# sisl/MADRL

Hardware: AMD Instinct MI355X
Metric: env-steps/sec at fixed batch (PursuitEvade 16x16, 8v30) (higher is better)
Workload: dtype u8/int32 grid state, f32 observations, f64 reward arithmetic; 1 GPU; PursuitEvade 16x16, 8 pursuers / 30 evaders, obs_range 7, rectangle_map, surround, n_catch 2, flatten, local reward, 65536 envs per GPU, horizon 500; envs_per_gpu=65536, envs_total=65536, parallelism=env-sharded x1, streams_per_gpu=2, rccl_ranks=1

## Files before the change

madrl_amd/csrc/pursuit_wave.hpp:

```cpp
#pragma once

#include <type_traits>

#include "common.hpp"
#include "pursuit_rules.hpp"
#include "pursuit_zm16.hpp"

namespace madrl {
namespace pw {

#ifndef MADRL_PW_WAVES
#define MADRL_PW_WAVES 5
#endif
#define MADRL_PW_OCC __attribute__((amdgpu_waves_per_eu(S::OCC, S::OCC)))

constexpr uint32_t SENT = 0xFFFFFFFFu;
constexpr uint32_t CAUGHT = 0x10000u;

struct WaveDev {
    int32_t n_catch, surround, reward_global, sample_maps, n_maps, max_steps, auto_reset;
    int32_t fmap_stride;
    int32_t max_opponents;
    int32_t reverse;
    uint32_t k0, k1, gid_base;
    double catchr, term_pursuit, urgency, cw;
    int64_t n_envs;
    const uint32_t *fmaps;
    const float *vtab;
    const int32_t *pending;
    const uint32_t *cnt_tmpl;
    const uint32_t *slot_tab;
    const double *cw_env;
    const double *catchr_env;
    uint8_t *state;
    uint32_t *flags;
    uint32_t *zmask;
};

struct WaveIO {
    const uint8_t *mask;
    const int32_t *inj_pos;
    const int32_t *inj_map;
    const int32_t *actions;
    const int32_t *inj_eact;
    float *obs;
    float *rew;
    uint8_t *done;
    int32_t *removed;
    int32_t flex;
    int32_t control_evaders;
    const float *obs_prev;
};

__device__ __forceinline__ double sload_f64(const double *p, int64_t index) {
    return ((const __attribute__((address_space(4))) double *)(uint64_t)p)[index];
}

struct KArgs {
    WaveDev d;
    WaveIO io;
};
typedef const __attribute__((address_space(4))) KArgs *KArgsPtr;
__device__ __forceinline__ KArgsPtr cold_args() { return kernargs<KArgs>(); }
__device__ __forceinline__ int32_t pending_count(int64_t env, int k) {
    const int32_t *pend = cold_args()->d.pending;
    return ((const __attribute__((address_space(4))) int32_t *)(uint64_t)pend)[2 * env + k];
}

template <int XS_, int YS_, int P_, int E_, int R_, int FLATTEN_>
struct Shape {
    static constexpr int XS = XS_, YS = YS_, P = P_, E = E_, A = P_ + E_, R = R_, FLATTEN = FLATTEN_;
    static constexpr int OFF = (R - 1) / 2;
    static constexpr int PAD = OFF > 1 ? OFF : 1;
    static constexpr int GW = YS + 2 * PAD;
    static constexpr int GH = XS + 2 * PAD;
    static constexpr int GSZ = (GH * GW + 3) / 4 * 4;
    static constexpr int D = FLATTEN ? 3 * R * R + 1 : 4 * R * R;
    static constexpr int DV = D / 4;
    static constexpr int NQ = P * DV;
    static constexpr int NS = (NQ + 63) / 64;
    static constexpr int MWORDS = 1;
    static constexpr bool ZM16 = zm16::eligible(P, R, FLATTEN);
    static constexpr int ZMW = ZM16 ? 32 : 64;
    static constexpr int OCC = NS <= 5 ? MADRL_PW_WAVES : (MADRL_PW_WAVES < 4 ? MADRL_PW_WAVES : 4);
    static constexpr int X_FILL = 3 * GSZ;
    static constexpr int X_SKIP = 3 * GSZ + 1;
    static constexpr int X_ID = 3 * GSZ + 2;
    static constexpr int X_VTAB = (X_ID + P + 3) / 4 * 4;
    static constexpr int NVT = 72;
    static constexpr int X_NEED = X_VTAB + NVT;
    static constexpr int X_OBSV = X_NEED + (XS * YS + 3) / 4;
    static constexpr int LDS_DWORDS = X_OBSV + (P + 3) / 4 * 4;
    static constexpr int NGW = (E + 31) / 32 > 0 ? (E + 31) / 32 : 1;
    static constexpr int NTW = (A + 31) / 32;
    static constexpr int OFF_GONE = (16 + 2 * A + 3) / 4 * 4;
    static constexpr int OFF_TERM = OFF_GONE + 4 * NGW;
    static constexpr int REC_BYTES = (OFF_TERM + 4 * NTW + 15) / 16 * 16;
    static constexpr int REC_DW = REC_BYTES / 4;
    static_assert(REC_DW <= 64, "the whole record must fit one dword per lane");
    static_assert(A <= 64, "one wavefront per env: n_pursuers + n_evaders must fit 64 lanes");
    static_assert(R % 2 == 1, "odd obs_range only (even ranges run on the generic kernel)");
    static_assert(D % 4 == 0, "observation row must be a whole number of float4");
    static_assert(LDS_DWORDS * 4 <= 64 * 1024, "LDS budget");
    static_assert(NS <= 8, "stale-zero mask: one bit per slot in each byte of the lane's mask dword");
    static constexpr bool LIVE = false;
    static constexpr bool TO = false;
    static constexpr bool H16 = false;
    static constexpr bool LEAN_REGS = false;
    static constexpr bool TABLED = false;
    static constexpr int X_TAB = 0;
};

template <int XS_, int YS_, int P_, int E_, int R_, int FLATTEN_>
struct LShape : Shape<XS_, YS_, P_, E_, R_, FLATTEN_> {
    static constexpr bool LIVE = true;
};
constexpr int NOT_HERE = 0xFF;

template <int XS_, int YS_, int P_, int E_, int R_, int FLATTEN_>
struct TShape : Shape<XS_, YS_, P_, E_, R_, FLATTEN_> {
    static constexpr bool TO = true;
};
template <int XS_, int YS_, int P_, int E_, int R_, int FLATTEN_>
struct TLShape : LShape<XS_, YS_, P_, E_, R_, FLATTEN_> {
    static constexpr bool TO = true;
};
template <int XS_, int YS_, int P_, int E_, int R_, int FLATTEN_>
struct THShape : Shape<XS_, YS_, P_, E_, R_, FLATTEN_> {
    static constexpr bool TO = true;
    static constexpr bool H16 = true;
    static constexpr bool LEAN_REGS = true;
};
template <int XS_, int YS_, int P_, int E_, int R_, int FLATTEN_>
struct TLHShape : LShape<XS_, YS_, P_, E_, R_, FLATTEN_> {
    static constexpr bool TO = true;
    static constexpr bool H16 = true;
    static constexpr bool LEAN_REGS = true;
};

__device__ __forceinline__ double pairwise8(const double *r) {
    return ((r[0] + r[1]) + (r[2] + r[3])) + ((r[4] + r[5]) + (r[6] + r[7]));
}

template <int P>
__device__ __forceinline__ double np_sum_regs(const double (&a)[P]) {
    if constexpr (P < 8) {
        double res = 0.0;
#pragma unroll
        for (int i = 0; i < P; ++i) res += a[i];
        return res;
    } else {
        double r[8];
#pragma unroll
        for (int i = 0; i < 8; ++i) r[i] = a[i];
        constexpr int LIM = P - (P % 8);
#pragma unroll
        for (int i = 8; i < LIM; i += 8) {
#pragma unroll
            for (int k = 0; k < 8; ++k) r[k] += a[i + k];
        }
        double res = pairwise8(r);
#pragma unroll
        for (int i = LIM; i < P; ++i) res += a[i];
        return res;
    }
}

template <int P>
__device__ __forceinline__ double np_sum_first(const double (&a)[P], int n) {
    double res = 0.0;
    if (n < 8) {
#pragma unroll
        for (int i = 0; i < (P < 8 ? P : 7); ++i)
            if (i < n) res += a[i];
        return res;
    }
    if constexpr (P >= 8) {
        double r[8];
#pragma unroll
        for (int i = 0; i < 8; ++i) r[i] = a[i];
        const int lim = n - (n % 8);
#pragma unroll
        for (int i = 8; i + 8 <= P; i += 8) {
            if (i < lim) {
#pragma unroll
                for (int k = 0; k < 8; ++k) r[k] += a[i + k];
            }
        }
        res = pairwise8(r);
#pragma unroll
        for (int i = 8; i < P; ++i)
            if (i >= lim && i < n) res += a[i];
    }
    return res;
}

typedef float v4f_t __attribute__((ext_vector_type(4)));
template <int I, int N, class F>
__device__ __forceinline__ void static_for(F &&f) {
    if constexpr (I < N) {
        f(std::integral_constant<int, I>{});
        static_for<I + 1, N>(f);
    }
}
template <int OFF, bool H16 = false>
__device__ __forceinline__ void store_slot_masked(const void *base, uint32_t voff, uint32_t v0, uint32_t v1, uint32_t v2, uint32_t v3,
                                                  v4f_t val, uint64_t m0, uint64_t m1, uint64_t m2, uint64_t m3, uint64_t m_nt) {
    static_assert(!H16, "store_slot_masked is float32 geometry: an H16 shape runs its in-place pass through half_slot_in_place");
    uint64_t sv;
    asm volatile("s_mov_b64 %0, exec\n\t"
                 "s_mov_b64 exec, %1\n\tglobal_store_dword %6, %7, %12 offset:%13\n\t"
                 "s_mov_b64 exec, %2\n\tglobal_store_dword %6, %8, %12 offset:%13+4\n\t"
                 "s_mov_b64 exec, %3\n\tglobal_store_dword %6, %9, %12 offset:%13+8\n\t"
                 "s_mov_b64 exec, %4\n\tglobal_store_dword %6, %10, %12 offset:%13+12\n\t"
                 "s_mov_b64 exec, %5\n\tglobal_store_dwordx4 %6, %11, %12 offset:%13 nt\n\t"
                 "s_mov_b64 exec, %0\n\ts_nop 0"
                 : "=&s"(sv) : "s"(m0), "s"(m1), "s"(m2), "s"(m3), "s"(m_nt), "v"(voff), "v"(v0), "v"(v1), "v"(v2), "v"(v3), "v"(val),
                   "s"(base), "n"(OFF));
}
__device__ __forceinline__ uint32_t quad_or(uint32_t v) {
    v |= (uint32_t)__builtin_amdgcn_update_dpp(0, (int)v, 0xB1, 0xF, 0xF, true);
    v |= (uint32_t)__builtin_amdgcn_update_dpp(0, (int)v, 0x4E, 0xF, 0xF, true);
    return v;
}

__device__ __forceinline__ void prefetch3(uint32_t &r0, uint32_t &r1, uint32_t &r2, const void *b0, uint32_t o0, const void *b1, uint32_t o1,
                                          const void *b2, uint32_t o2) {
    asm volatile("s_nop 4\n\tglobal_load_dword %0, %3, %4\n\tglobal_load_dword %1, %5, %6\n\tglobal_load_dword %2, %7, %8"
                 : "=&v"(r0), "=&v"(r1), "=&v"(r2) : "v"(o0), "s"(b0), "v"(o1), "s"(b1), "v"(o2), "s"(b2));
}
template <int N>
__device__ __forceinline__ void prefetch_wait(uint32_t &r0, uint32_t &r1, uint32_t &r2) {
    static_assert(N >= 0 && N < 64, "vmcnt is a 6-bit field");
    asm volatile("s_waitcnt vmcnt(%3)" : "+v"(r0), "+v"(r1), "+v"(r2) : "n"(N) : "memory");
}

template <class RowPtr>
__device__ __forceinline__ void half_slot_in_place(RowPtr row, uint32_t slot, bool valid, uint32_t keep4, uint32_t v0, uint32_t v1, uint32_t v2,
                                                   uint32_t v3) {
    typedef __attribute__((address_space(1))) uint64_t gu64_t;
    if (!valid) return;
    auto hb = [](uint32_t v) -> uint64_t { return half_bits(__uint_as_float((uint32_t)max((int)v, 0))); };
    uint64_t w = hb(v0) | (hb(v1) << 16) | (hb(v2) << 32) | (hb(v3) << 48);
    gu64_t *const at = reinterpret_cast<gu64_t *>(row) + slot;
    if (keep4 != 0u) {
        const uint64_t old = __hip_atomic_load(at, __ATOMIC_RELAXED, __HIP_MEMORY_SCOPE_AGENT);
        const uint64_t k = ((keep4 & 0x00000001u) ? 0x000000000000FFFFull : 0ull) | ((keep4 & 0x00000100u) ? 0x00000000FFFF0000ull : 0ull) |
                           ((keep4 & 0x00010000u) ? 0x0000FFFF00000000ull : 0ull) | ((keep4 & 0x01000000u) ? 0xFFFF000000000000ull : 0ull);
        w = (w & ~k) | (old & k);
    }
    *at = w;
}

template <int LN>
__device__ __forceinline__ void put_lane(uint32_t &w, uint32_t v) {
    const uint32_t sv = (uint32_t)__builtin_amdgcn_readfirstlane((int)v);
    asm("v_writelane_b32 %0, %1, %2" : "+v"(w) : "s"(sv), "n"(LN));
}
template <int LN, int END>
__device__ __forceinline__ void put_zero_from(uint32_t &w) {
    if constexpr (LN < END) {
        put_lane<LN>(w, 0u);
        put_zero_from<LN + 1, END>(w);
    }
}

template <class S, int NT>
struct Fill {
    static constexpr int NEEDW = (S::XS * S::YS + 3) / 4;
    static constexpr int TABW = S::TABLED ? 2 * S::DV : 0;
    static constexpr int J_MAP = (S::GSZ + NT - 1) / NT;
    static constexpr int J_NEED = 2 * J_MAP;
    static constexpr int J_VT = J_NEED + (NEEDW + NT - 1) / NT;
    static constexpr int J_TAB = J_VT + (S::NVT + NT - 1) / NT;
    static constexpr int J_END = J_TAB + (TABW + NT - 1) / NT;
    static constexpr int first(int j) { return j < J_MAP ? 0 : j < J_NEED ? J_MAP : j < J_VT ? J_NEED : j < J_TAB ? J_VT : J_TAB; }
    static constexpr int words(int j) { return j < J_NEED ? S::GSZ : j < J_VT ? NEEDW : j < J_TAB ? S::NVT : TABW; }
};
template <class S, int NT, int J>
__device__ __forceinline__ uint32_t fill_load(uint32_t utid, const uint32_t *cnt, const uint32_t *map, const uint32_t *vtab, const uint32_t *tab) {
    using F = Fill<S, NT>;
    constexpr int t = J - F::first(J), n = F::words(J);
    const uint32_t k = utid + (uint32_t)(NT * t);
    const uint32_t kc = (NT * (t + 1) <= n) ? k : (k < (uint32_t)n ? k : (uint32_t)n - 1u);
    if constexpr (J < F::J_MAP) return cnt[kc];
    else if constexpr (J < F::J_NEED) return map[kc];
    else if constexpr (J < F::J_VT) return map[(uint32_t)S::GSZ + kc];
    else if constexpr (J < F::J_TAB) return vtab[kc];
    else return tab[kc];
}
template <class S, int NT, int J, bool FIRST>
__device__ __forceinline__ void fill_store(uint32_t *L, uint32_t utid, uint32_t v) {
    using F = Fill<S, NT>;
    constexpr int t = J - F::first(J), n = F::words(J);
    const uint32_t k = utid + (uint32_t)(NT * t);
    if ((NT * (t + 1) <= n) || k < (uint32_t)n) {
        if constexpr (J < F::J_MAP) {
            L[S::GSZ + k] = v;
            L[2 * S::GSZ + k] = v;
        } else if constexpr (J < F::J_NEED) L[k] = v;
        else if constexpr (J < F::J_VT) L[S::X_NEED + k] = v;
        else if constexpr (J < F::J_TAB) L[S::X_VTAB + k] = v;
        else L[S::X_TAB + k] = v;
    }
    if constexpr (FIRST && J == F::J_MAP) {
        if (utid == 0u) {
            L[S::X_FILL] = v;
            L[S::X_SKIP] = SENT;
        }
    }
}
template <int N>
__device__ __forceinline__ void staged_wait(uint32_t *a) {
    if constexpr (N >= 8) {
        asm volatile("" : "+v"(a[N - 1]), "+v"(a[N - 2]), "+v"(a[N - 3]), "+v"(a[N - 4]), "+v"(a[N - 5]), "+v"(a[N - 6]), "+v"(a[N - 7]), "+v"(a[N - 8]));
        staged_wait<N - 8>(a);
    } else if constexpr (N >= 4) {
        asm volatile("" : "+v"(a[N - 1]), "+v"(a[N - 2]), "+v"(a[N - 3]), "+v"(a[N - 4]));
        staged_wait<N - 4>(a);
    } else if constexpr (N >= 2) {
        asm volatile("" : "+v"(a[N - 1]), "+v"(a[N - 2]));
        staged_wait<N - 2>(a);
    } else if constexpr (N == 1) {
        asm volatile("" : "+v"(a[0]));
    }
}
template <class S, int NT, int J0, int J1, int CAP, bool FIRST>
__device__ __forceinline__ void fill_trips(uint32_t *L, uint32_t utid, const uint32_t *cnt, const uint32_t *map, const uint32_t *vtab, const uint32_t *tab) {
    if constexpr (J0 < J1) {
        constexpr int JB = J0 + CAP < J1 ? J0 + CAP : J1;
        uint32_t st[JB - J0];
        static_for<J0, JB>([&](auto jc) {
            if constexpr (decltype(jc)::value == JB - 1) __builtin_amdgcn_sched_barrier(0);
            st[decltype(jc)::value - J0] = fill_load<S, NT, decltype(jc)::value>(utid, cnt, map, vtab, tab);
        });
        staged_wait<JB - J0>(st);
        static_for<J0, JB>([&](auto jc) { fill_store<S, NT, decltype(jc)::value, FIRST>(L, utid, st[decltype(jc)::value - J0]); });
        fill_trips<S, NT, JB, J1, CAP, FIRST>(L, utid, cnt, map, vtab, tab);
    }
}
constexpr int FILL_FIRST = 56, FILL_BATCH = 16;

#ifndef MADRL_ABLATE
#define MADRL_ABLATE 0
#endif
#ifndef MADRL_PW_EXP
#define MADRL_PW_EXP 0
#endif

template <class S, int MODE, bool INJECT, bool CTRL = false>
__global__ __launch_bounds__(64) MADRL_PW_OCC void pursuit_wave_kernel(const WaveDev d, const WaveIO io) {
    static_assert(!CTRL || (S::E >= S::P && (MODE == 0 || INJECT)), "evader control: n_evaders >= n_pursuers, flexible instantiation");
    static_assert(!CTRL || !S::LIVE, "evader control has no per-env agent counts");
    static_assert(!S::TO || (MODE == 1 && INJECT && !CTRL), "the two-buffer step: the flexible step kernel only");
    static_assert(!S::H16 || S::TO, "binary16 buffers: the two-buffer step only");
    constexpr int P = S::P, E = S::E, A = S::A, GW = S::GW, PAD = S::PAD, GSZ = S::GSZ, NS = S::NS;
    __shared__ __attribute__((aligned(16))) uint32_t L[S::LDS_DWORDS];
    const int lane = threadIdx.x;
    const uint32_t ulane = threadIdx.x;
    const bool is_p = lane < P;
    const int eslot = lane - P;

#if MADRL_PW_EXP & 4
    if (d.n_envs > 0) return;
#endif
    using F = Fill<S, 64>;
    const int n_envs = (int)d.n_envs, stride = (int)gridDim.x;
    if (n_envs <= 0) return;
    auto phys = [&](int e) -> int64_t { return (int64_t)(d.reverse ? n_envs - 1 - e : e); };
    auto zm_env = [](int64_t env) -> int64_t { return (MADRL_ABLATE & (256 | 512)) ? (env & 255) : env; };
    const uint32_t zm_lane = S::ZM16 ? (ulane & 31u) : ulane;
    [[maybe_unused]] const uint32_t zm_keep = S::ZM16 ? zm16::keep_low(P, S::R, lane) : 0u;
    const uint32_t *const vtab_u = reinterpret_cast<const uint32_t *>(d.vtab);
    constexpr int ROOM = FILL_FIRST - 6 * NS - 3;
    constexpr int JF = F::J_END < (ROOM > 4 ? ROOM : 4) ? F::J_END : (ROOM > 4 ? ROOM : 4);
    const uint32_t rec_off = (ulane < (uint32_t)S::REC_DW ? ulane : (uint32_t)S::REC_DW - 1u) * 4u;
    const uint32_t act_off = (ulane < (uint32_t)P ? ulane : (uint32_t)P - 1u) * 4u;
    uint32_t st[JF], sraw[6 * NS];
    static_for<0, JF>([&](auto jc) { st[decltype(jc)::value] = fill_load<S, 64, decltype(jc)::value>(ulane, d.cnt_tmpl, d.fmaps, vtab_u, nullptr); });
#pragma unroll
    for (int k = 0; k < 6 * NS; ++k) sraw[k] = d.slot_tab[64u * k + ulane];
    uint32_t cur_rec, cur_zm;
    int cur_act = 4;
    __builtin_amdgcn_sched_barrier(0);
    {
        const int64_t env0 = phys((int)blockIdx.x < n_envs ? (int)blockIdx.x : n_envs - 1);
        cur_rec = *reinterpret_cast<const uint32_t *>(d.state + env0 * (int64_t)S::REC_BYTES + rec_off);
        if constexpr (MODE == 1) cur_act = *reinterpret_cast<const int *>(reinterpret_cast<const char *>(io.actions + env0 * P) + act_off);
        cur_zm = d.zmask[zm_env(env0) * S::ZMW + zm_lane];
    }
    asm volatile("" : "+v"(cur_rec), "+v"(cur_act), "+v"(cur_zm));
    staged_wait<6 * NS>(sraw);
    staged_wait<JF>(st);
    static_for<0, JF>([&](auto jc) { fill_store<S, 64, decltype(jc)::value, true>(L, ulane, st[decltype(jc)::value]); });
    fill_trips<S, 64, JF, F::J_END, FILL_BATCH, true>(L, ulane, d.cnt_tmpl, d.fmaps, vtab_u, nullptr);
    if (lane < P) L[S::X_ID + lane] = __float_as_uint((float)((double)lane / (double)P));
    if (ulane >= (uint32_t)S::REC_DW) cur_rec = 0u;
    if (!is_p) cur_act = 4;
    int s_cst[NS][4];
    int s_rel3[NS];
    int s_src[NS];
#pragma unroll
    for (int s = 0; s < NS; ++s) {
#pragma unroll
        for (int k = 0; k < 4; ++k) s_cst[s][k] = (int)sraw[6 * s + k] * 4;
        s_rel3[s] = (int)sraw[6 * s + 4];
        s_src[s] = (int)sraw[6 * s + 5] * 4;
    }
    int cached_map = 0;
    int cached_np = P;
    const uint8_t *need_tab = reinterpret_cast<const uint8_t *>(&L[S::X_NEED]);
    uint32_t *const layer = &L[is_p ? GSZ : 2 * GSZ];
    const int rec_src0 = (lane >= 4 ? 2 * (lane - 4) : 0) * 4, rec_src1 = rec_src0 + 4;

    auto isP = [&]() { return fresh(lane) < P; };
    auto isE = [&]() { return (unsigned)(fresh(lane) - P) < (unsigned)E; };
    auto isAgent = [&]() { return fresh(lane) < A; };
    auto fetch_rec = [&](int64_t env) -> uint32_t {
        return (fresh(lane) < S::REC_DW) ? uniform_ptr(reinterpret_cast<const uint32_t *>(d.state + env * (int64_t)S::REC_BYTES))[ulane] : 0u;
    };
    auto fetch_act = [&](int64_t env) -> int {
        if constexpr (MODE == 1) return isP() ? uniform_ptr(io.actions + env * P)[ulane] : 4;
        else return 4;
    };
    auto fetch_zm = [&](int64_t env) -> uint32_t {
        if constexpr (S::LEAN_REGS) return uniform_ptr(d.zmask + zm_env(env) * S::ZMW)[S::ZM16 ? ((uint32_t)fresh(lane) & 31u) : (uint32_t)fresh(lane)];
        else return uniform_ptr(d.zmask + zm_env(env) * S::ZMW)[zm_lane];
    };
    wave_sync();
#if MADRL_PW_EXP & 8
    if (d.n_envs > 0) { if (s_cst[0][0] + s_cst[NS - 1][3] + s_rel3[0] + s_src[NS - 1] + (int)cur_rec == 0x12345) io.rew[0] = 1.f; return; }
#endif

    constexpr bool PIPE = (MODE == 1) && !INJECT && !(MADRL_ABLATE & (1 | 8 | 16 | 64));
    constexpr int VM_PER_ENV = 5 * NS + 6 - ((MADRL_ABLATE & 512) ? 1 : 0);
    static_assert(!PIPE || VM_PER_ENV < 64, "vmcnt range");
    for (int e = blockIdx.x; e < n_envs; e += stride) {
        const int64_t env = phys(e);
        const bool has_next = e + stride < n_envs;
        const int64_t nenv = phys(has_next ? e + stride : e);
        uint32_t nxt_rec = 0, nxt_zm = 0xFFFFFFFFu;
        int nxt_act = 4;
        uint32_t pf_rec, pf_act, pf_zm;
        if constexpr (PIPE) {
            prefetch3(pf_rec, pf_act, pf_zm, d.state + nenv * (int64_t)S::REC_BYTES, rec_off, io.actions + nenv * P, act_off,
                      d.zmask + zm_env(nenv) * S::ZMW, zm_lane * 4u);
        } else {
#if MADRL_ABLATE & 64
            nxt_rec = cur_rec ^ (uint32_t)(fresh(lane) == 0);
            nxt_act = cur_act;
#else
            if (has_next) {
                nxt_rec = fetch_rec(nenv);
                nxt_act = fetch_act(nenv);
                nxt_zm = fetch_zm(nenv);
            }
#endif
        }
        bool skip = false;
        if constexpr (MODE == 0) skip = (io.mask != nullptr && io.mask[env] == 0);
        if (!skip) {
            uint32_t tick = __builtin_amdgcn_readlane(cur_rec, 0);
            int32_t tstep = (int32_t)__builtin_amdgcn_readlane(cur_rec, 1);
            int32_t map_id = (int32_t)__builtin_amdgcn_readlane(cur_rec, 2);
            const uint32_t xyw = (uint32_t)__shfl((int)cur_rec, 4 + (lane >> 1));
            const pr::Cell at = pr::unpack_xy(xyw, lane & 1);
            int x = at.x, y = at.y;
            uint64_t gone = (uint32_t)__builtin_amdgcn_readlane(cur_rec, S::OFF_GONE / 4);
            if constexpr (S::NGW > 1) gone |= (uint64_t)(uint32_t)__builtin_amdgcn_readlane(cur_rec, S::OFF_GONE / 4 + 1) << 32;
            uint64_t term = (uint32_t)__builtin_amdgcn_readlane(cur_rec, S::OFF_TERM / 4);
            if constexpr (S::NTW > 1) term |= (uint64_t)(uint32_t)__builtin_amdgcn_readlane(cur_rec, S::OFF_TERM / 4 + 1) << 32;
            const uint32_t gid = d.gid_base + (uint32_t)env;
            const uint32_t k0 = fresh_s(d.k0), k1 = fresh_s(d.k1);
            int np = P, ne = E;
            if constexpr (S::LIVE) {
                const bool here = x != NOT_HERE;
                np = __popcll(__builtin_amdgcn_ballot_w64(isP() && here));
                ne = __popcll(__builtin_amdgcn_ballot_w64(isE() && here));
                if (!here) {
                    x = 0;
                    y = 0;
                }
            }
            auto isLP = [&]() {
                if constexpr (S::LIVE) return fresh(lane) < np;
                else return isP();
            };
            bool do_reset = (MODE == 0);
            uint32_t done_bits = 0;
            float rew_out = 0.0f;
            int n_removed = 0;
            bool alive = isLP() || (isE() && !((gone >> eslot) & 1ull));
            int cell = (x + PAD) * GW + y + PAD;

            auto load_map = [&](int mid) {
                if (cached_map == mid) return;
                const KArgsPtr ka = cold_args();
                fill_trips<S, 64, F::J_MAP, F::J_VT, FILL_BATCH, false>(L, ulane, nullptr, ka->d.fmaps + (int64_t)mid * ka->d.fmap_stride, nullptr, nullptr);
                cached_map = mid;
                wave_sync();
            };
            load_map(map_id);

            if constexpr (MODE == 1) {
                const bool e_alive = alive && !isP();
                if (e_alive) atomicAdd(&layer[cell], 1u);
                wave_sync();
                int kpre = 0;
                if (isP()) {
                    const pr::Clip4 n = pr::clipped_neighbours<GW, S::XS, S::YS>(x, y);
                    const uint32_t *ec = &L[2 * GSZ];
                    kpre = (int)(ec[cell - n.dxm] + ec[cell + n.dxp] + ec[cell + n.dyp] + ec[cell - n.dym]);
                }
                wave_sync();
                if (e_alive) atomicSub(&layer[cell], 1u);
                const int kidx = __popcll((~gone) & ((1ull << (eslot & 63)) - 1ull));
                int act = cur_act;
                bool injected = false;
                if constexpr (CTRL) {
                    const int from_k = __builtin_amdgcn_ds_bpermute((kidx < P ? kidx : 0) * 4, cur_act);
                    injected = io.inj_eact != nullptr;
                    int pact;
                    if (injected) pact = isP() ? io.inj_eact[env * P + lane] : 4;
                    else pact = pr::pursuer_action(gid, tick, (uint32_t)lane, k0, k1);
                    act = isP() ? pact : (kidx < P ? from_k : 4);
                    injected = true;
                } else if constexpr (INJECT) {
                    injected = io.inj_eact != nullptr;
                    if (injected && e_alive) act = io.inj_eact[env * E + kidx];
                }
                if (!injected) {
#if MADRL_ABLATE & 4
                    u32x4 r; r.x = (gid * 2654435761u + tick * 40503u + (uint32_t)kidx * 2246822519u) ^ k0 ^ k1;
#else
                    const u32x4 r = philox4x32_10(gid, tick, (uint32_t)kidx, TAG_EVADER_ACT, k0, k1);
#endif
                    if (!isP()) act = (int)__umulhi(r.x, 5u);
                }
                const int dcell = pr::move_dcell<GW>(act);
                const bool tflag = (term >> lane) & 1ull;
                const bool in_building = L[cell] != 0u;
                const bool target_free = L[cell + dcell] == 0u;
                const bool newterm = alive && !tflag && in_building;
                if (alive && !tflag && !in_building && target_free) {
                    cell += dcell;
                    x += pr::move_dx(act), y += pr::move_dy(act);
                }
                term |= __ballot(newterm);
                if (alive) atomicAdd(&layer[cell], 1u);
                wave_sync();
                bool caught = false;
                if (e_alive) {
                    const uint32_t *pc = &L[GSZ];
                    if (d.surround) caught = pr::cells_with_pursuers(pc[cell - GW], pc[cell + GW], pc[cell + 1], pc[cell - 1], SENT) == (int)need_tab[x * S::YS + y];
                    else caught = (int)pc[cell] >= d.n_catch;
                    if (caught) atomicAdd(&layer[cell], CAUGHT);
                }
                const uint64_t caught_mask = __ballot(caught) >> P;
                gone |= caught_mask;
                wave_sync();
                double r = 0.0;
                if (isLP()) {
                    const uint32_t *ec = &L[2 * GSZ];
                    bool sur;
                    if (d.surround) sur = pr::caught_beside(ec[cell - GW], ec[cell + GW], ec[cell + 1], ec[cell - 1], SENT, CAUGHT);
                    else sur = ec[cell] >= CAUGHT;
                    double catchr = d.catchr;
                    if constexpr (INJECT) { if (d.catchr_env != nullptr) catchr = sload_f64(d.catchr_env, env); }
                    r = pr::pursuer_reward(catchr, kpre, d.term_pursuit, sur, d.urgency);
                }
                if (d.reward_global) {
                    double all[P];
#pragma unroll
                    for (int k = 0; k < P; ++k) {
                        if constexpr (S::LEAN_REGS) {
                            const uint64_t rb = __builtin_bit_cast(uint64_t, r);
                            const uint32_t rl = (uint32_t)__builtin_amdgcn_ds_bpermute(4 * k, (int)(uint32_t)rb);
                            const uint32_t rh = (uint32_t)__builtin_amdgcn_ds_bpermute(4 * k, (int)(uint32_t)(rb >> 32));
                            all[k] = __builtin_bit_cast(double, ((uint64_t)rh << 32) | rl);
                        } else {
                            all[k] = __shfl(r, k);
                        }
                    }
                    if constexpr (S::LIVE) r = isLP() ? np_sum_first<P>(all, np) / (double)np : 0.0;
                    else r = np_sum_regs<P>(all) / (double)P;
                }
                tick += 1;
                tstep += 1;
                constexpr uint64_t all_e = (1ull << E) - 1ull;
                if ((gone & all_e) == all_e) done_bits |= 1u;
                if (d.max_steps > 0 && tstep >= d.max_steps) done_bits |= 2u;
                do_reset = d.auto_reset && done_bits != 0;
                rew_out = (float)r;
                n_removed = __popcll(caught_mask);
            }

            if constexpr (!PIPE) asm volatile("" : "+v"(nxt_rec), "+v"(nxt_act), "+v"(nxt_zm));
            uint32_t zm = cur_zm;
            if constexpr (S::ZM16) zm = zm16::unpack(fresh(lane) < 32 ? cur_zm : cur_zm >> 16, zm_keep);

            const int npass = (MODE == 1 && do_reset) ? 2 : 1;
            for (int pass = 0; pass < npass; ++pass) {
                if (do_reset && pass == npass - 1) {
                    gone = 0ull;
                    term = 0ull;
                    const KArgsPtr ka = cold_args();
                    const double cw = ka->d.cw_env != nullptr ? sload_f64(ka->d.cw_env, env) : ka->d.cw;
                    const int max_opponents = ka->d.max_opponents;
                    bool inj_map = false, inj_pos = false;
                    if constexpr (MODE == 0) {
                        inj_map = io.inj_map != nullptr;
                        inj_pos = io.inj_pos != nullptr;
                    }
                    if (inj_map) {
                        map_id = __builtin_amdgcn_readfirstlane(io.inj_map[env]);
                    } else if (ka->d.sample_maps) {
                        const u32x4 rm = philox4x32_10(gid, tick, 0u, TAG_RESET_ENV, k0, k1);
                        map_id = (int)__umulhi(rm.x, (uint32_t)ka->d.n_maps);
                    }
                    load_map(map_id);
                    const pr::Window win = pr::reset_window(gid, tick, k0, k1, cw, S::XS, S::YS);
                    int n_create = E;
                    if constexpr (S::LIVE) {
                        const pr::Counts live = pr::clamp_pending(pending_count(env, 0), pending_count(env, 1), P, E);
                        np = live.np, ne = n_create = live.ne;
                    }
                    if (max_opponents > 0 && !inj_pos) n_create = pr::reset_n_create(gid, tick, k0, k1, max_opponents, S::LIVE ? ne : E);
                    bool exists = false;
                    if (isAgent()) {
                        if constexpr (S::LIVE) exists = isLP() || (!isP() && eslot < n_create);
                        else exists = isP() || eslot < n_create;
                        if (inj_pos) {
                            x = io.inj_pos[(env * A + lane) * 2];
                            y = io.inj_pos[(env * A + lane) * 2 + 1];
                            if (!isP() && x < 0) exists = false;
                        } else {
                            for (uint32_t att = 0; att < 1024u; ++att) {
                                const uint32_t aidx = S::LIVE ? (uint32_t)(isP() ? lane : np + eslot) : (uint32_t)lane;
                                const u32x4 rp = philox4x32_10(gid, tick, aidx, TAG_RESET_POS | (att << 8), k0, k1);
                                x = win.xlb + (int)__umulhi(rp.x, (uint32_t)(win.xub - win.xlb));
                                y = win.ylb + (int)__umulhi(rp.y, (uint32_t)(win.yub - win.ylb));
                                if (L[(x + PAD) * GW + y + PAD] == 0u) break;
                            }
                        }
                        if (exists) {
                            cell = (x + PAD) * GW + y + PAD;
                            atomicAdd(&layer[cell], 1u);
                        } else {
                            x = 0;
                            y = 0;
                        }
                    }
                    gone = __ballot(isE() && !exists) >> P;
                    alive = exists;
                    tick += 1;
                    tstep = 0;
                    wave_sync();
                }
                if constexpr (S::LIVE) {
                    if (np != cached_np) {
                        if (lane < P) L[S::X_ID + lane] = __float_as_uint((float)((double)lane / (double)np));
                        cached_np = np;
                        wave_sync();
                    }
                }
                uint32_t cnt = 0;
                if (alive) cnt = layer[cell] & 0xFFFFu;
                wave_sync();
                if (alive) layer[cell] = L[S::X_VTAB + cnt];
                wave_sync();
#if MADRL_ABLATE & 8
                if (d.n_envs < 0)
#endif
                {
                    int origin = isP() ? ((x - S::OFF + PAD) * GW + (y - S::OFF + PAD)) * 4 : 0;
                    int n_rows = P;
                    if constexpr (CTRL) {
                        const uint64_t obsv = ~gone & ((1ull << P) - 1ull);
                        n_rows = __popcll(obsv);
                        const bool is_obs = isE() && eslot < P && ((obsv >> (eslot & 63)) & 1ull);
                        if (is_obs) L[S::X_OBSV + __popcll(obsv & ((1ull << (eslot & 63)) - 1ull))] = (uint32_t)(((x - S::OFF + PAD) * GW + (y - S::OFF + PAD)) * 4);
                        wave_sync();
                        origin = (isP() && lane < n_rows) ? (int)L[S::X_OBSV + lane] : 0;
                    }
                    if constexpr (S::LIVE) n_rows = np;
                    const char *orow_u = (const char *)uniform_ptr(io.obs + env * (int64_t)(P * S::D));
                    asm volatile("s_nop 4" : "+s"(orow_u));
                    const uint32_t voff = ulane * 16u;
                    [[maybe_unused]] const auto prow_g = uniform_ptr(S::TO ? io.obs_prev + env * (int64_t)(P * S::D / (S::H16 ? 2 : 1)) : io.obs);
                    [[maybe_unused]] const auto orow_g = uniform_ptr(io.obs + env * (int64_t)(P * S::D / (S::H16 ? 2 : 1)));
                    const char *Lb = reinterpret_cast<const char *>(L);
                    auto cell_at = [&](int off) -> uint32_t { return *reinterpret_cast<const uint32_t *>(Lb + off); };
                    uint32_t acc = 0u;
                    if constexpr (S::H16) {
                        if (pass == 1) asm volatile("s_waitcnt vmcnt(0)" ::: "memory");
                    }
                    [[maybe_unused]] uint32_t to_need[S::TO ? NS : 1], to_bits[S::TO && !S::H16 ? NS : 1];
                    static_for<0, NS>([&](auto sc) {
                        constexpr int s = decltype(sc)::value;
                        const int base = __builtin_amdgcn_ds_bpermute(s_src[s], origin);
                        const uint32_t v0 = cell_at(base + s_cst[s][0]);
                        const uint32_t v1 = cell_at(base + s_cst[s][1]);
                        const uint32_t v2 = cell_at(base + s_cst[s][2]);
                        const uint32_t v3 = cell_at((int)__umul24((uint32_t)base, (uint32_t)s_rel3[s]) + s_cst[s][3]);
                        const uint32_t top = __builtin_amdgcn_perm(v1, v0, 0x0C0C0703u) | __builtin_amdgcn_perm(v3, v2, 0x07030C0Cu);
                        const uint32_t out4 = (top >> 7) & 0x01010101u;
                        const uint32_t nz4 = ((top >> 5) | (top >> 6)) & 0x01010101u;
                        const uint32_t old4 = (zm >> (NS - 1 - s)) & 0x01010101u;
                        const uint32_t dirty = out4 & old4;
                        if constexpr (S::TO) {
                            if (pass == 0) {
                                bool row_live = true;
                                if constexpr (S::LIVE) row_live = (s_src[s] >> 2) < n_rows;
                                const bool in_row = (64 * (s + 1) <= S::NQ) ? true : (fresh(lane) + 64 * s < S::NQ);
                                const uint32_t need4 = in_row ? (row_live ? dirty : 0x01010101u) : 0u;
                                to_need[s] = need4;
                                if constexpr (S::H16) {
                                    if constexpr (s == 0) to_bits[0] = ~need4 & ~out4 & nz4;
                                    else to_bits[0] |= (~need4 & ~out4 & nz4) << s;
                                } else {
                                    to_bits[s] = ~need4 & ~out4 & nz4;
                                }
                                return;
                            }
                        }
                        bool valid = (64 * (s + 1) <= S::NQ) ? true : (fresh(lane) + 64 * s < S::NQ);
                        if constexpr (CTRL || S::LIVE) {
                            const bool row_live = (s_src[s] >> 2) < n_rows;
                            acc = (acc << 1) | (row_live ? ((out4 & old4) | (~out4 & nz4)) : old4);
                            valid = valid && row_live;
                        } else {
                            acc = (acc << 1) | ((out4 & old4) | (~out4 & nz4));
                        }
                        bool clean = dirty == 0u;
#if MADRL_ABLATE & 1
                        valid = d.n_envs < 0;
#endif
#if MADRL_ABLATE & (2 | 512)
                        clean = true;
#endif
                        const uint32_t st = valid ? (clean ? 0u : dirty) : 0x80000000u;
#if MADRL_ABLATE & 32
                        {
                            uint32_t burn = acc;
                            asm volatile("v_xor_b32 %0, %0, %1\n v_xor_b32 %0, %0, %1\n v_xor_b32 %0, %0, %1\n v_xor_b32 %0, %0, %1\n v_xor_b32 %0, %0, %1\n"
                                         "v_xor_b32 %0, %0, %1\n v_xor_b32 %0, %0, %1\n v_xor_b32 %0, %0, %1\n v_xor_b32 %0, %0, %1\n v_xor_b32 %0, %0, %1\n"
                                         "v_xor_b32 %0, %0, %1\n v_xor_b32 %0, %0, %1\n v_xor_b32 %0, %0, %1\n v_xor_b32 %0, %0, %1\n v_xor_b32 %0, %0, %1\n"
                                         "v_xor_b32 %0, %0, %1\n v_xor_b32 %0, %0, %1\n v_xor_b32 %0, %0, %1\n v_xor_b32 %0, %0, %1\n v_xor_b32 %0, %0, %1"
                                         : "+v"(burn) : "v"(v0));
                            acc = burn;
                        }
#endif
#if MADRL_ABLATE & 128
                        {
                            uint32_t sburn = fresh_s(0u);
                            asm volatile("s_add_u32 %0, %0, 1\n s_add_u32 %0, %0, 1\n s_add_u32 %0, %0, 1\n s_add_u32 %0, %0, 1\n s_add_u32 %0, %0, 1\n"
                                         "s_add_u32 %0, %0, 1\n s_add_u32 %0, %0, 1\n s_add_u32 %0, %0, 1\n s_add_u32 %0, %0, 1\n s_add_u32 %0, %0, 1\n"
                                         "s_add_u32 %0, %0, 1\n s_add_u32 %0, %0, 1\n s_add_u32 %0, %0, 1\n s_add_u32 %0, %0, 1\n s_add_u32 %0, %0, 1\n"
                                         "s_add_u32 %0, %0, 1\n s_add_u32 %0, %0, 1\n s_add_u32 %0, %0, 1\n s_add_u32 %0, %0, 1\n s_add_u32 %0, %0, 1"
                                         : "+s"(sburn) : : "scc");
                        }
#endif
                        if constexpr (S::H16) {
                            half_slot_in_place(orow_g, 64u * s + ulane, valid, clean ? 0u : dirty, v0, v1, v2, v3);
                        } else {
                            const void *sb = orow_u + 4096 * (s / 4);
                            const uint32_t lim = (uint32_t)fresh((st - 1u < 0x01010101u) ? (int)SENT : 0);
                            const uint32_t grp = quad_or(st == 0u ? (out4 ^ 0x01010101u) : 0u);
                            const uint32_t nt = (uint32_t)fresh(st == 0u ? (int)grp : 0);
                            const v4f_t val = {__uint_as_float((uint32_t)max((int)v0, 0)), __uint_as_float((uint32_t)max((int)v1, 0)),
                                               __uint_as_float((uint32_t)max((int)v2, 0)), __uint_as_float((uint32_t)max((int)v3, 0))};
                            store_slot_masked<1024 * (s % 4), S::H16>(sb, voff, v0, v1, v2, v3, val, __builtin_amdgcn_ballot_w64(v0 < lim),
                                                              __builtin_amdgcn_ballot_w64(v1 < lim), __builtin_amdgcn_ballot_w64(v2 < lim),
                                                              __builtin_amdgcn_ballot_w64(v3 < lim), __builtin_amdgcn_ballot_w64(nt != 0u));
                        }
                    });
                    if constexpr (S::TO) {
                        if (pass == 0) {
                            typedef uint32_t v4u_t __attribute__((ext_vector_type(4)));
                            typedef __attribute__((address_space(1))) v4u_t gv4u_t;
                            typedef __attribute__((address_space(1))) v4f_t gv4f_t;
                            constexpr int TG = NS <= 5 ? NS : 4;
                            typedef uint32_t v2u_t __attribute__((ext_vector_type(2)));
                            typedef __attribute__((address_space(1))) v2u_t gv2u_t;
                            using old_t = std::conditional_t<S::H16, uint64_t, v4u_t>;
                            using gold_t = std::conditional_t<S::H16, __attribute__((address_space(1))) uint64_t, gv4u_t>;
                            auto emit = [&](auto sc, const old_t oldv) {
                                constexpr int s = decltype(sc)::value;
                                const int base = __builtin_amdgcn_ds_bpermute(s_src[s], origin);
                                const uint32_t need4 = to_need[s];
                                uint32_t w0 = (uint32_t)max((int)cell_at(base + s_cst[s][0]), 0);
                                uint32_t w1 = (uint32_t)max((int)cell_at(base + s_cst[s][1]), 0);
                                uint32_t w2 = (uint32_t)max((int)cell_at(base + s_cst[s][2]), 0);
                                uint32_t w3 = (uint32_t)max((int)cell_at((int)__umul24((uint32_t)base, (uint32_t)s_rel3[s]) + s_cst[s][3]), 0);
                                if constexpr (S::H16) {
                                    const bool in_row = (64 * (s + 1) <= S::NQ) ? true : (fresh(lane) + 64 * s < S::NQ);
                                    const uint32_t oldx = (uint32_t)oldv, oldy = (uint32_t)(oldv >> 32);
                                    uint32_t lo = (uint32_t)half_bits(__uint_as_float(w0)) | ((uint32_t)half_bits(__uint_as_float(w1)) << 16);
                                    uint32_t hi = (uint32_t)half_bits(__uint_as_float(w2)) | ((uint32_t)half_bits(__uint_as_float(w3)) << 16);
                                    const uint32_t klo = ((need4 & 0x00000001u) ? 0x0000FFFFu : 0u) | ((need4 & 0x00000100u) ? 0xFFFF0000u : 0u);
                                    const uint32_t khi = ((need4 & 0x00010000u) ? 0x0000FFFFu : 0u) | ((need4 & 0x01000000u) ? 0xFFFF0000u : 0u);
                                    lo = (lo & ~klo) | (oldx & klo);
                                    hi = (hi & ~khi) | (oldy & khi);
                                    const uint32_t oldnz = ((oldx & 0xFFFFu) != 0u ? 0x00000001u : 0u) | ((oldx >> 16) != 0u ? 0x00000100u : 0u) |
                                                           ((oldy & 0xFFFFu) != 0u ? 0x00010000u : 0u) | ((oldy >> 16) != 0u ? 0x01000000u : 0u);
                                    acc = (acc << 1) | ((to_bits[0] >> s) & 0x01010101u) | (need4 & oldnz);
                                    if (in_row) __builtin_nontemporal_store(v2u_t{lo, hi}, reinterpret_cast<gv2u_t *>(orow_g) + (64u * s + ulane));
                                } else {
                                    if (need4 & 0x00000001u) w0 = oldv.x;
                                    if (need4 & 0x00000100u) w1 = oldv.y;
                                    if (need4 & 0x00010000u) w2 = oldv.z;
                                    if (need4 & 0x01000000u) w3 = oldv.w;
                                    const uint32_t oldnz = (oldv.x != 0u ? 0x00000001u : 0u) | (oldv.y != 0u ? 0x00000100u : 0u) |
                                                           (oldv.z != 0u ? 0x00010000u : 0u) | (oldv.w != 0u ? 0x01000000u : 0u);
                                    acc = (acc << 1) | to_bits[s] | (need4 & oldnz);
                                    const bool in_row = (64 * (s + 1) <= S::NQ) ? true : (fresh(lane) + 64 * s < S::NQ);
                                    if (in_row) {
                                        const v4f_t wv = {__uint_as_float(w0), __uint_as_float(w1), __uint_as_float(w2), __uint_as_float(w3)};
                                        __builtin_nontemporal_store(wv, reinterpret_cast<gv4f_t *>(orow_g) + (64u * s + ulane));
                                    }
                                }
                            };
                            static_for<0, (NS + TG - 1) / TG>([&](auto gc) {
                                constexpr int g0 = decltype(gc)::value * TG, g1 = g0 + TG < NS ? g0 + TG : NS;
                                uint32_t any = 0u;
#pragma unroll
                                for (int s = g0; s < g1; ++s) any |= to_need[s];
                                if (__builtin_amdgcn_ballot_w64(any != 0u) != 0ull) {
                                    old_t old[TG];
#pragma unroll
                                    for (int s = g0; s < g1; ++s) {
                                        old[s - g0] = old_t{};
                                        if (to_need[s] != 0u) old[s - g0] = reinterpret_cast<const gold_t *>(prow_g)[64u * s + ulane];
                                    }
                                    static_for<g0, g1>([&](auto sc) { emit(sc, old[decltype(sc)::value - g0]); });
                                } else {
                                    static_for<g0, g1>([&](auto sc) { emit(sc, old_t{}); });
                                }
                            });
                        }
                    }
                    zm = acc;
                }
                wave_sync();
                if (alive) layer[cell] = 0u;
                wave_sync();
            }
#if MADRL_ABLATE & 16
            if (d.n_envs < 0)
#endif
            if constexpr (MODE == 1) {
                if (isP()) uniform_ptr(io.rew + env * P)[ulane] = rew_out;
                if (fresh(lane) == 0) {
                    io.done[env] = (uint8_t)done_bits;
                    io.removed[env] = n_removed;
                    cold_args()->d.flags[env] = done_flag_word(done_bits);
                }
            }
            {
                int myxy = x | (y << 8);
                if constexpr (S::LIVE) {
                    if (!(isP() ? isLP() : eslot < ne)) myxy = NOT_HERE | (NOT_HERE << 8);
                }
                [[maybe_unused]] auto src_of = [&](auto kc) -> int {
                    if constexpr (S::LEAN_REGS) return ((fresh(lane) >= 4 ? 2 * (fresh(lane) - 4) : 0) + decltype(kc)::value) * 4;
                    else return decltype(kc)::value ? rec_src1 : rec_src0;
                };
                const uint32_t lo = (uint32_t)__builtin_amdgcn_ds_bpermute(src_of(std::integral_constant<int, 0>{}), myxy);
                const uint32_t hi = (uint32_t)__builtin_amdgcn_ds_bpermute(src_of(std::integral_constant<int, 1>{}), myxy);
                uint32_t w = (lo & 0xFFFFu) | (hi << 16);
                put_lane<0>(w, tick);
                put_lane<1>(w, (uint32_t)tstep);
                put_lane<2>(w, (uint32_t)map_id);
                put_lane<3>(w, 0u);
                put_lane<S::OFF_GONE / 4>(w, (uint32_t)gone);
                if constexpr (S::NGW > 1) put_lane<S::OFF_GONE / 4 + 1>(w, (uint32_t)(gone >> 32));
                put_lane<S::OFF_TERM / 4>(w, (uint32_t)term);
                if constexpr (S::NTW > 1) put_lane<S::OFF_TERM / 4 + 1>(w, (uint32_t)(term >> 32));
                put_zero_from<S::OFF_TERM / 4 + S::NTW, S::REC_DW>(w);
#if MADRL_ABLATE & 16
                if (d.n_envs < 0)
#endif
                if (fresh(lane) < S::REC_DW)
                    uniform_ptr(reinterpret_cast<uint32_t *>(d.state + env * (int64_t)S::REC_BYTES))[ulane] = w;
#if MADRL_ABLATE & 16
                if (d.n_envs < 0)
#endif
#if !(MADRL_ABLATE & 512)
                if constexpr (S::ZM16) {
                    const uint32_t h = zm16::pack(zm, zm_keep);
                    const uint32_t other = __builtin_amdgcn_permlane32_swap(h, h, false, false)[1];
                    if (fresh(lane) < 32) uniform_ptr(d.zmask + zm_env(env) * S::ZMW)[ulane] = h | (other << 16);
                } else {
                    uniform_ptr(d.zmask + zm_env(env) * 64)[ulane] = zm;
                }
#endif
            }
        }
        if constexpr (PIPE) {
            prefetch_wait<VM_PER_ENV>(pf_rec, pf_act, pf_zm);
            nxt_rec = (fresh(lane) < S::REC_DW) ? pf_rec : 0u;
            nxt_act = (int)pf_act;
            nxt_zm = pf_zm;
        }
        cur_rec = nxt_rec;
        cur_act = nxt_act;
        cur_zm = nxt_zm;
    }
}

template <class S>
void wave_to_launch(const WaveDev &d, const WaveIO &io, int64_t blocks, hipStream_t s);
template <class S>
void wave_to_f16_launch(const WaveDev &d, const WaveIO &io, int64_t blocks, hipStream_t s);

}
}
```

madrl_amd/pursuit.py:

```python
import ctypes as C

import numpy as np
import torch

from . import _lib
from .base import AbstractMAEnv, Agent, SingleEnvDelegate
from .maps import as_map_pool
from .spaces import Box, Discrete

_DEFAULTS = dict(
    sample_maps=False, reward_mech="global", n_evaders=1, n_pursuers=1, obs_range=3,
    flatten=True, layer_norm=10, n_catch=2, random_opponents=False, max_opponents=10,
    catchr=0.01, caughtr=-0.01, term_pursuit=5.0, term_evade=-5.0, urgency_reward=0.0,
    include_id=True, train_pursuit=True, initial_config=None, surround=True,
    constraint_window=1.0, curriculum_remove_every=500, curriculum_constrain_rate=0.0,
    curriculum_turn_off_shaping=np.inf)


class PursuitAgent(Agent):

    def __init__(self, obs_shape):
        self._obs_shape = tuple(obs_shape)

    @property
# ... 25 lines not shown
        for k in list(kwargs):
            if k in ("ally_layer", "opponent_layer", "evader_controller", "pursuer_controller"):
                raise ValueError("%s is a Python object hook of the reference; the batched engine "
                                 "injects evader actions through step(..., evader_actions=)" % k)
            if k not in kw:
                raise TypeError("unknown PursuitEvade kwarg %r" % k)
            kw[k] = kwargs[k]
        if kw["random_opponents"] and int(kw["max_opponents"]) < 2:
            raise ValueError("random_opponents draws randint(1, max_opponents): max_opponents must be >= 2")
        if not kw["train_pursuit"]:
            if kw["random_opponents"]:
                raise NotImplementedError("train_pursuit=False with random_opponents (a per-reset number of pursuers, :180-181)")
            if int(kw["n_evaders"]) < int(kw["n_pursuers"]):
                raise ValueError("train_pursuit=False: collect_obs indexes evaders_gone[i] for i < n_pursuers (:418-428); "
                                 "the reference raises IndexError in reset() when n_evaders < n_pursuers")
            if per_env_counts:
                raise NotImplementedError("per_env_counts=True with train_pursuit=False (evader control) is not supported")
        for k, v in kw.items():
            if k == "reward_mech":
                self._reward_mech = v
            else:
                setattr(self, k, v)
        self.map_pool = as_map_pool(map_pool)
        self.map_matrix = self.map_pool[0]
        self.xs, self.ys = self.map_matrix.shape
        self.obs_offset = int((self.obs_range - 1) / 2)
        self.n_envs = int(n_envs)
        self.device = torch.device(device)
        self._seed_value = int(seed)
        self.env_id_base = int(env_id_base)
        self.max_steps = int(max_steps)
        self.auto_reset = bool(auto_reset)
        self._threads, self._max_blocks = int(threads), int(max_blocks)
        self._handle = None
        self.setup()

    def _config(self):
        c = _lib.PursuitConfig()
        c.struct_size = C.sizeof(_lib.PursuitConfig)
        c.xs, c.ys = self.xs, self.ys
        c.n_pursuers, c.n_evaders = int(self.n_pursuers), int(self.n_evaders)
        c.obs_range, c.n_catch = int(self.obs_range), int(self.n_catch)
        c.surround, c.flatten, c.include_id = int(bool(self.surround)), int(bool(self.flatten)), int(bool(self.include_id))
        c.reward_global = int(self._reward_mech == "global")
        c.sample_maps, c.n_maps = int(bool(self.sample_maps)), int(self.map_pool.shape[0])
        c.max_steps, c.auto_reset = self.max_steps, int(self.auto_reset)
        c.max_opponents = int(self.max_opponents) if self.random_opponents else 0
        c.control_evaders = int(not self.train_pursuit)
        c.catchr, c.term_pursuit = float(self.catchr), float(self.term_pursuit)
        c.urgency_reward, c.layer_norm = float(self.urgency_reward), float(self.layer_norm)
        c.constraint_window = float(self.constraint_window)
        c.seed, c.env_id_base = self._seed_value, self.env_id_base
        return c

    def setup(self):
        L = _lib.lib()
        if self.device.type != "cuda":
            raise _lib.MadrlError("BatchedPursuitEvade needs a ROCm device (got %s); there is no "
                                  "CPU path" % self.device)
        cfg = self._config()
        dim = C.c_int32()
        _lib.check(L.madrl_pursuit_obs_dim(C.byref(cfg), C.byref(dim)))
        nbytes, rbytes = C.c_uint64(), C.c_int32()
        _lib.check(L.madrl_pursuit_state_bytes(C.byref(cfg), self.n_envs, C.byref(nbytes)))
        _lib.check(L.madrl_pursuit_record_bytes(C.byref(cfg), C.byref(rbytes)))
        self.record_bytes = rbytes.value
        foff = C.c_uint64()
        _lib.check(L.madrl_pursuit_flags_offset(C.byref(cfg), self.n_envs, C.byref(foff)))
        N, P, E, D = self.n_envs, int(self.n_pursuers), int(self.n_evaders), dim.value
        shape_key = (N, P, E, D, nbytes.value)
        if getattr(self, "_shape_key", None) != shape_key:
            dev = self.device
            self._state = torch.zeros(nbytes.value, dtype=torch.uint8, device=dev)
            self._obs = torch.zeros((N, P, D), dtype=self.obs_dtype, device=dev)
            self._half_pair = (self._obs, torch.zeros_like(self._obs)) if self._half else None
            self._obs32 = None
            self._rew = torch.zeros((N, P), dtype=torch.float32, device=dev)
            self._done = torch.zeros(N, dtype=torch.uint8, device=dev)
            self._removed = torch.zeros(N, dtype=torch.int32, device=dev)
            self._flags = self._state[foff.value:foff.value + 4 * N].view(N, 4)
            self._flag_views = tuple(self._flags[:, k].view(torch.bool) for k in range(3))
            self._shape_key = shape_key
            self._obs_is_fresh = True
            self._obs_version = None
        self.obs_dim = D
        self._destroy()
        h = C.c_void_p()
        dev_index = self.device.index if self.device.index is not None else torch.cuda.current_device()
        _lib.check(L.madrl_pursuit_create(C.byref(cfg), self.map_pool.ctypes.data_as(C.c_void_p), N,
                                          dev_index, _lib.ptr(self._state), C.byref(h)))
        self._handle = h
        self._handle_key = self._create_key()
        if getattr(self, "_obs_is_fresh", False) and not self._half:
            _lib.check(L.madrl_pursuit_declare_obs_zero(h, _lib.ptr(self._obs), _lib.current_stream(self.device)))
        self.handle_generation = getattr(self, "handle_generation", 0) + 1
        if self.per_env_counts:
            if getattr(self, "_pending", None) is None or self._pending.shape[0] != N or self._pending_cap != (P, E):
                self._pending = torch.tensor([P, E], dtype=torch.int32, device=self.device).repeat(N, 1).contiguous()
                self._pending_cap = (P, E)
            _lib.check(L.madrl_pursuit_set_agent_counts(h, _lib.ptr(self._pending)))
        if getattr(self, "_cw_env", None) is not None and self._cw_env.shape[0] == N:
            _lib.check(L.madrl_pursuit_set_curriculum(h, _lib.ptr(self._cw_env), _lib.ptr(self._catchr_env)))
        else:
            self._cw_env = self._catchr_env = None
        if self._threads or self._max_blocks:
            _lib.check(L.madrl_pursuit_set_launch(h, self._threads, self._max_blocks))
        if getattr(self, "_kernel", "auto") != "auto":
            self.set_kernel(self._kernel)
        elif N >= 4096:
            self._hint_fast_path()
        if getattr(self, "_walk", "auto") != "auto":
            self.set_walk(self._walk)
        obs_shape = (D,) if self.flatten else (self.obs_range, self.obs_range, 4)
        self.pursuers = [PursuitAgent(obs_shape) for _ in range(P)]
        self.act_dims = [5] * P

    _hinted = set()

    def _hint_fast_path(self):
        from . import build as _build
        shape = (self.xs, self.ys, int(self.n_pursuers), int(self.n_evaders), int(self.obs_range), int(bool(self.flatten)))
        if shape in BatchedPursuitEvade._hinted or self.kernel_kind != "generic" or not self.train_pursuit and shape[2] + shape[3] > 64:
            return
        if self.per_env_counts:
            lines = _build.pursuit_live_lines(*shape, include_id=bool(self.include_id))
            if lines is not None:
                import warnings
                BatchedPursuitEvade._hinted.add(shape)
                warnings.warn("PursuitEvade per-env agent counts at capacity %d v %d (%dx%d, obs_range %d) run on the generic kernel; the line "
                              "%s in madrl_amd/csrc/pursuit_live_specializations.def (and a rebuild: `python -m madrl_amd.build "
                              "--pursuit-live-shape %s`) gives them the %s kernel"
                              % (shape[2], shape[3], shape[0], shape[1], shape[4], lines[0].replace(" ", ""), " ".join(str(v) for v in shape),
                                 "one-wavefront" if lines[0].startswith("XL(") else "multi-wavefront"), stacklevel=3)
                return
            lines = _build.pursuit_live_crowd_lines(*shape, include_id=bool(self.include_id))
            if lines is not None:
                import warnings
                BatchedPursuitEvade._hinted.add(shape)
                warnings.warn("PursuitEvade per-env agent counts at capacity %d v %d (%dx%d, obs_range %d) run on the generic kernel; the line "
                              "%s in madrl_amd/csrc/pursuit_live_specializations.def (and a rebuild: `python -m madrl_amd.build "
                              "--pursuit-live-crowd-shape %s`) gives them the crowd kernel"
                              % (shape[2], shape[3], shape[0], shape[1], shape[4], lines[0].replace(" ", ""), " ".join(str(v) for v in shape)),
                              stacklevel=3)
            return
        kind, _ = _build.pursuit_fast_path(*shape, include_id=bool(self.include_id))
        if kind is None and self.train_pursuit and _build.pursuit_crowd_path(*shape, include_id=bool(self.include_id))[0] is not None:
            import warnings
            BatchedPursuitEvade._hinted.add(shape)
            warnings.warn("PursuitEvade %dx%d, %d v %d, obs_range %d runs on the generic kernel; `python -m madrl_amd.build --pursuit-crowd-shape "
                          "%s` compiles the crowd kernel for this shape (results are identical, a step takes less time)"
                          % (shape[0], shape[1], shape[2], shape[3], shape[4], " ".join(str(v) for v in shape)), stacklevel=3)
            return
        if kind is not None:
            import warnings
            BatchedPursuitEvade._hinted.add(shape)
            warnings.warn("PursuitEvade %dx%d, %d v %d, obs_range %d runs on the generic kernel; `python -m madrl_amd.build --pursuit-shape %s` "
                          "compiles the specialised kernel for this shape (results are identical, a step takes about half the time)"
                          % (shape[0], shape[1], shape[2], shape[3], shape[4], " ".join(str(v) for v in shape)), stacklevel=3)

    def set_kernel(self, kind):
        k = {"auto": _lib.KERNEL_AUTO, "generic": _lib.KERNEL_GENERIC, "wave": _lib.KERNEL_WAVE}[kind]
        _lib.check(_lib.lib().madrl_pursuit_set_kernel(self._handle, k))
        self._kernel = kind

    @property
    def kernel_kind(self):
        out = C.c_int32()
# ... 511 lines not shown
```

Before: 1.124 billion env-steps/s.

## Skip zero-fill stores over observation slots already known to be zero

For 16-bit zero-mask shapes on the in-place float32 path, the per-slot non-temporal group store mask is now built from the old and new zero state. Groups that were and remain zero are no longer rewritten, which cuts global memory store traffic for observations. The zero-mask prefetch lane indexing and the mask merge with zm_keep change to carry this extra state. The Python side now records the obs tensor version at allocation. The risk is stale data if the zero tracking ever diverges from the buffer contents.

```diff
diff --git a/madrl_amd/csrc/pursuit_wave.hpp b/madrl_amd/csrc/pursuit_wave.hpp
--- a/madrl_amd/csrc/pursuit_wave.hpp
+++ b/madrl_amd/csrc/pursuit_wave.hpp
@@ -82,6 +82,7 @@
     static constexpr int MWORDS = 1;
     static constexpr bool ZM16 = zm16::eligible(P, R, FLATTEN);
     static constexpr int ZMW = ZM16 ? 32 : 64;
+    static constexpr bool ZSKIP = ZM16;
     static constexpr int OCC = NS <= 5 ? MADRL_PW_WAVES : (MADRL_PW_WAVES < 4 ? MADRL_PW_WAVES : 4);
     static constexpr int X_FILL = 3 * GSZ;
     static constexpr int X_SKIP = 3 * GSZ + 1;
@@ -120,20 +121,24 @@
 template <int XS_, int YS_, int P_, int E_, int R_, int FLATTEN_>
 struct TShape : Shape<XS_, YS_, P_, E_, R_, FLATTEN_> {
     static constexpr bool TO = true;
+    static constexpr bool ZSKIP = false;
 };
 template <int XS_, int YS_, int P_, int E_, int R_, int FLATTEN_>
 struct TLShape : LShape<XS_, YS_, P_, E_, R_, FLATTEN_> {
     static constexpr bool TO = true;
+    static constexpr bool ZSKIP = false;
 };
 template <int XS_, int YS_, int P_, int E_, int R_, int FLATTEN_>
 struct THShape : Shape<XS_, YS_, P_, E_, R_, FLATTEN_> {
     static constexpr bool TO = true;
+    static constexpr bool ZSKIP = false;
     static constexpr bool H16 = true;
     static constexpr bool LEAN_REGS = true;
 };
 template <int XS_, int YS_, int P_, int E_, int R_, int FLATTEN_>
 struct TLHShape : LShape<XS_, YS_, P_, E_, R_, FLATTEN_> {
     static constexpr bool TO = true;
+    static constexpr bool ZSKIP = false;
     static constexpr bool H16 = true;
     static constexpr bool LEAN_REGS = true;
 };
@@ -217,6 +222,12 @@
                  "s_mov_b64 exec, %0\n\ts_nop 0"
                  : "=&s"(sv) : "s"(m0), "s"(m1), "s"(m2), "s"(m3), "s"(m_nt), "v"(voff), "v"(v0), "v"(v1), "v"(v2), "v"(v3), "v"(val),
                    "s"(base), "n"(OFF));
+}
+template <uint32_t K>
+__device__ __forceinline__ uint32_t add_here(uint32_t a) {
+    uint32_t r;
+    asm volatile("v_add_u32 %0, %1, %2" : "=v"(r) : "n"(K), "v"(a));
+    return r;
 }
 __device__ __forceinline__ uint32_t quad_or(uint32_t v) {
     v |= (uint32_t)__builtin_amdgcn_update_dpp(0, (int)v, 0xB1, 0xF, 0xF, true);
@@ -354,6 +365,7 @@
     static_assert(!CTRL || !S::LIVE, "evader control has no per-env agent counts");
     static_assert(!S::TO || (MODE == 1 && INJECT && !CTRL), "the two-buffer step: the flexible step kernel only");
     static_assert(!S::H16 || S::TO, "binary16 buffers: the two-buffer step only");
+    static_assert(!S::ZSKIP || (S::ZM16 && !S::TO && !S::H16), "zeros over known zeros: the in-place float32 pass of a 16-bit-mask shape only");
     constexpr int P = S::P, E = S::E, A = S::A, GW = S::GW, PAD = S::PAD, GSZ = S::GSZ, NS = S::NS;
     __shared__ __attribute__((aligned(16))) uint32_t L[S::LDS_DWORDS];
     const int lane = threadIdx.x;
@@ -444,7 +456,7 @@
         uint32_t pf_rec, pf_act, pf_zm;
         if constexpr (PIPE) {
             prefetch3(pf_rec, pf_act, pf_zm, d.state + nenv * (int64_t)S::REC_BYTES, rec_off, io.actions + nenv * P, act_off,
-                      d.zmask + zm_env(nenv) * S::ZMW, zm_lane * 4u);
+                      d.zmask + zm_env(nenv) * S::ZMW, (S::ZSKIP ? ((uint32_t)fresh(lane) & 31u) : zm_lane) * 4u);
         } else {
 #if MADRL_ABLATE & 64
             nxt_rec = cur_rec ^ (uint32_t)(fresh(lane) == 0);
@@ -598,6 +610,7 @@
             if constexpr (!PIPE) asm volatile("" : "+v"(nxt_rec), "+v"(nxt_act), "+v"(nxt_zm));
             uint32_t zm = cur_zm;
             if constexpr (S::ZM16) zm = zm16::unpack(fresh(lane) < 32 ? cur_zm : cur_zm >> 16, zm_keep);
+            if constexpr (S::ZSKIP) zm |= add_here<0x01010101u>(zm_keep);
 
             const int npass = (MODE == 1 && do_reset) ? 2 : 1;
             for (int pass = 0; pass < npass; ++pass) {
@@ -725,13 +738,13 @@
                             }
                         }
                         bool valid = (64 * (s + 1) <= S::NQ) ? true : (fresh(lane) + 64 * s < S::NQ);
+                        uint32_t new4 = (out4 & old4) | (~out4 & nz4);
                         if constexpr (CTRL || S::LIVE) {
                             const bool row_live = (s_src[s] >> 2) < n_rows;
-                            acc = (acc << 1) | (row_live ? ((out4 & old4) | (~out4 & nz4)) : old4);
+                            new4 = row_live ? new4 : old4;
                             valid = valid && row_live;
-                        } else {
-                            acc = (acc << 1) | ((out4 & old4) | (~out4 & nz4));
                         }
+                        acc = (acc << 1) | new4;
                         bool clean = dirty == 0u;
 #if MADRL_ABLATE & 1
                         valid = d.n_envs < 0;
@@ -766,8 +779,19 @@
                         } else {
                             const void *sb = orow_u + 4096 * (s / 4);
                             const uint32_t lim = (uint32_t)fresh((st - 1u < 0x01010101u) ? (int)SENT : 0);
-                            const uint32_t grp = quad_or(st == 0u ? (out4 ^ 0x01010101u) : 0u);
-                            const uint32_t nt = (uint32_t)fresh(st == 0u ? (int)grp : 0);
+                            uint32_t nt;
+                            if constexpr (S::ZSKIP) {
+#if MADRL_ABLATE & 1024
+                                const uint32_t x = ~out4 & nz4;
+#else
+                                const uint32_t x = old4 | new4;
+#endif
+                                const uint32_t grp = quad_or(st == 0u ? x : 0u);
+                                nt = (uint32_t)fresh(st == 0u ? (int)grp : 0);
+                            } else {
+                                const uint32_t grp = quad_or(st == 0u ? (out4 ^ 0x01010101u) : 0u);
+                                nt = (uint32_t)fresh(st == 0u ? (int)grp : 0);
+                            }
                             const v4f_t val = {__uint_as_float((uint32_t)max((int)v0, 0)), __uint_as_float((uint32_t)max((int)v1, 0)),
                                                __uint_as_float((uint32_t)max((int)v2, 0)), __uint_as_float((uint32_t)max((int)v3, 0))};
                             store_slot_masked<1024 * (s % 4), S::H16>(sb, voff, v0, v1, v2, v3, val, __builtin_amdgcn_ballot_w64(v0 < lim),
@@ -841,6 +865,7 @@
                         }
                     }
                     zm = acc;
+                    if constexpr (S::ZSKIP) zm |= add_here<0x01010101u>(zm_keep);
                 }
                 wave_sync();
                 if (alive) layer[cell] = 0u;
diff --git a/madrl_amd/pursuit.py b/madrl_amd/pursuit.py
--- a/madrl_amd/pursuit.py
+++ b/madrl_amd/pursuit.py
@@ -131,7 +131,7 @@
             self._flag_views = tuple(self._flags[:, k].view(torch.bool) for k in range(3))
             self._shape_key = shape_key
             self._obs_is_fresh = True
-            self._obs_version = None
+            self._obs_version = self._version_of_obs()
         self.obs_dim = D
         self._destroy()
         h = C.c_void_p()
```

New measurement: 1.153 billion env-steps/s (median of 6 runs). 1.03x the previous value.
